# Ryan-Faulkner/Simultaneous-Diffusion-for-Pointclouds

Hardware: AMD Instinct MI355X
Metric: Langevin denoising steps/sec on 64×1024 range images, 1/2/4/8 MI355X (higher is better)
Workload: dtype fp32x3; 1 GPU; Line.yml simultaneous sampling step (score-net fwd + Langevin update + consistency merge), 64x1024x2 range images; views_per_gpu=4, megabatch_views=4, mode=viewsplit, conv_arithmetic=fp32x3, parallelism=views1

## Files before the change

simultaneous-diffusion-for-pointclouds_amd/csrc/conv_kernel.h:

```cpp
#pragma once
#include <type_traits>

#include "common.h"

namespace sdp {

#ifndef SDP_KO
#define SDP_KO 0
#endif

#ifndef SDP_DMA_AUX
#define SDP_DMA_AUX 0
#endif
#ifndef SDP_STORE_AUX
#define SDP_STORE_AUX 0
#endif
#ifndef SDP_STORE_AUX16
#define SDP_STORE_AUX16 SDP_STORE_AUX
#endif

#ifndef SDP_S2_RING
#define SDP_S2_RING 4
#endif

#ifndef SDP_ROWS
#define SDP_ROWS 1
#endif

#ifdef SDP_TIMING
#define SDP_T(i) do { if (tid == 0) tclk[i] = __builtin_amdgcn_s_memtime(); } while (0)
#else
#define SDP_T(i) do { } while (0)
#endif

constexpr int PSTRIDE = 144;

template <int WM, int TC, int KS, int NW = 4, int NJ = 4, bool IO16 = false>
struct ConvTile {
  static constexpr int NTH = 64 * NW;
  static constexpr int WN = NW / WM;
  static constexpr int RW = 128 / TC;
  static constexpr int TR = WM * RW;
  static constexpr int NTILE = WN * 16 * NJ;
  static constexpr int WPC = 4 * (NJ == 2 ? 2 : 1) / NW;
  static constexpr int HALO = KS == 3 ? 1 : 0;
  static constexpr int PC = TC + 2 * HALO;
  static constexpr int PR = TR + 2 * HALO;
  static constexpr int NPIX = PR * PC;
  static constexpr int UPP = IO16 ? 4 : 8;
  static constexpr int NU = (NPIX * UPP + NTH - 1) / NTH;
  static constexpr int PATCH_BYTES = NU * (NTH / UPP) * PSTRIDE;
  static constexpr int RAW_BYTES = NU * NTH * 16;
  static constexpr int PIPE_BYTES = 2 * PATCH_BYTES + RAW_BYTES;
  static constexpr int EPI_BYTES = WM * 64 * (NTILE + 8) * 4;
  static constexpr int LDS_BYTES = PIPE_BYTES > EPI_BYTES ? PIPE_BYTES : EPI_BYTES;
  static_assert(LDS_BYTES * WPC <= 160 * 1024, "LDS budget (WPC workgroups per CU)");
};

SDP_DEV float4 ld4(const float* p) { return *reinterpret_cast<const float4*>(p); }

template <int NU, int NT, int NSTG_ = 5>
struct XformPlan {
  static constexpr int tap_of(int k) { return k * NT / NU; }
  static constexpr int first(int tap) {
    int k = 0;
    while (k < NU && tap_of(k) < tap) ++k;
    return k;
  }
  static constexpr int count(int tap) {
    int n = 0;
    for (int k = 0; k < NU; ++k) n += tap_of(k) == tap ? 1 : 0;
    return n;
  }
  static constexpr int max_count() {
    int m = 0;
    for (int t = 0; t < NT; ++t) m = count(t) > m ? count(t) : m;
    return m;
  }
  static constexpr int NSTG = NSTG_;
// ... 18 lines not shown
    if (kw < 2 && (blk == 8 || blk == 10)) return 4 * 0 + 2 * (blk == 10 ? 1 : 0) + 1;
  } else {
    if (kw < 2 && blk >= 4) return 4 * (1 + (blk - 4) / 2) + 2 * lo + 1;
  }
  return -1;
}
constexpr bool rows_plan_ok() {
  for (int kw = 0; kw < 3; ++kw)
    for (int row = 0; row < 10; ++row)
      for (int lo = 0; lo < 2; ++lo) {
        int n = (kw == 0 && row < 4) ? 1 : 0, at = -1;
        for (int o = 0; o < 9; ++o)
          for (int blk = 0; blk < 16; ++blk) {
            const int c = rows_read(o, blk);
            if (c >= 0 && o / 3 + (c & 1) == kw && c / 4 == row && ((c >> 1) & 1) == lo) {
              ++n;
              at = 16 * o + blk;
            }
          }
        if (n != 1) return false;
        const int kh0 = row > 7 ? row - 7 : 0, mb0 = row - kh0;
        if (at >= 16 * (3 * kw + kh0) + (mb0 < 4 ? mb0 : 4 + mb0)) return false;
        const int pkw = row == 9 ? kw : kw - 1, prow = row == 9 ? 0 : row + 1;
        if (pkw < 0) continue;
        if (rows_slot(pkw, prow) != rows_slot(kw, row)) return false;
        const int kh1 = prow < 2 ? prow : 2, mb1 = prow - kh1;
        if (at < 16 * (3 * pkw + kh1) + (mb1 < 4 ? 4 + mb1 : 8 + mb1)) return false;
      }
  return true;
}
static_assert(rows_plan_ok(), "A-fragment ring: a row is read once, between its slot's last use and its own first");

template <int MODE, int WM, int TC, int KS, bool POOL, bool ZP, bool PELU, int SH = 32, int NW = 4, bool TRN = false,
          int NJ = 4, bool IO16 = false, bool S2 = false>
__global__ __launch_bounds__(64 * NW, NJ == 2 ? 2 : 1) void conv_mfma_kernel(ConvArgs a) {
#if defined(__HIP_DEVICE_COMPILE__)
  static_assert(!IO16 || MODE == MODE_BF16, "the bf16 tape runs in bf16 mode");
  constexpr int ES = IO16 ? 2 : 4;
  constexpr int CPU = IO16 ? 8 : 4;
  constexpr int USH = IO16 ? 2 : 3;
  constexpr int PPU = CPU / 2;
  constexpr bool COPY = IO16 && !PELU;
  static_assert((SH == 32) == (MODE == MODE_F32), "bf16 modes: 16x16 shape; exact fp32: 32x32");
  static_assert(NW == 4 || (SH == 16 && !POOL), "2-wave workgroups: the 16x16 non-pooled forward only");
  static_assert(NJ == 4 || (SH == 16 && !POOL && KS == 3 && WM == 1), "32-Cout waves: the 16x16 3x3 tiles only");
  static_assert(!S2 || (NJ == 2 && NW == 4 && TC == 16 && ZP && !TRN && !IO16), "4x4 stride-2: zero-padded 32-Cout-wave tiles");
  using T = ConvTile<WM, TC, KS, NW, NJ, IO16>;
  constexpr int NTH = T::NTH;
  constexpr int NT = S2 ? 4 : KS * KS;
  constexpr bool TRANS = TRN && SH == 16 && !POOL;
  constexpr int NU = T::NU;
  constexpr int XT = NT >= 4 ? 4 : NT;
  constexpr bool ROWS = SDP_ROWS && SH == 16 && !S2 && NT == 9 && TC == 16 && NJ == 2 && !TRANS;
  __shared__ __attribute__((aligned(16))) char lds[T::LDS_BYTES];
  char* const raw = lds + 2 * T::PATCH_BYTES;

  const int tid = threadIdx.x, lane = tid & 63, wave = tid >> 6;
#ifdef SDP_TIMING
  unsigned long long tclk[8] = {0, 0, 0, 0, 0, 0, 0, 0};
  unsigned long long tbar = 0;
  const unsigned long long rt0 = __builtin_amdgcn_s_memrealtime();
#endif
  SDP_T(0);
  const int wm = WM == 1 ? 0 : (wave & 1), wn = WM == 1 ? wave : (wave >> 1);
  const int d = S2 ? 2 : a.dil, Hs = a.H / d, Ws = a.W / d;
  const int tiles_c = Ws / TC, tiles_rc = (Hs / T::TR) * tiles_c;
  const int nwg = gridDim.x;
  int t = (nwg & 7) ? (int)blockIdx.x : ((int)blockIdx.x & 7) * (nwg >> 3) + ((int)blockIdx.x >> 3);
  const int cblk = a.cpair ? (t & 1) : (int)blockIdx.y;
  if (a.cpair) t >>= 1;
  const int b = t / a.tiles_per_img;
  const int tile = t - b * a.tiles_per_img;
  t = tile;
  const int ph = t / tiles_rc;
  t -= ph * tiles_rc;
  const int ph_r = ph / d, ph_c = ph - (ph / d) * d;
  int trow, tcol;
  if (a.strip_w) {
    const int R = Hs / T::TR, sw = a.strip_w;
    const int strip = t / (R * sw), w_ = t - strip * (R * sw);
    trow = w_ / sw;
    tcol = strip * sw + (w_ - trow * sw);
  } else {
    trow = t / tiles_c;
    tcol = t % tiles_c;
  }
  const int sr0 = trow * T::TR, sc0 = tcol * TC;
  const int n0 = cblk * T::NTILE;
  const int wrow0 = wm * T::RW;

  const int Cin = a.Cin, Cout = a.Cout;
  const int nck = Cin / 32;
  const int nchunks = S2 ? 4 * nck : nck;
  const int NB = Cout / 32;
  const int f0 = n0 / 16 + wn * NJ;
  const int nbg0 = f0 / 2;

  f32x16 acc[4][2];
  f32x4 acc4[8][NJ];
  if constexpr (SH == 32) {
    static_for<0, 4>([&](auto i) {
      static_for<0, 2>([&](auto j) {
#pragma unroll
        for (int r = 0; r < 16; ++r) acc[i][j][r] = 0.f;
      });
    });
// ... 53 lines not shown
    if constexpr (S2) return (c >= 2 * nck ? c - 2 * nck : c) >> 1;
    else return c;
  };
  auto chunk_soff = [&](int c) __attribute__((always_inline)) {
    if constexpr (S2) {
      c = min(c, nchunks - 1);
      const int rho = c >= 2 * nck ? 1 : 0, r = c - rho * 2 * nck;
      return ((rho * a.W + (r & 1)) * Cin + (r >> 1) * 32) * ES;
    } else {
      return c * 32 * ES;
    }
  };
  const int my_cv = tid & (T::UPP - 1);
  float4 ssv[2][PPU];
  auto load_ss = [&](auto buf, int chunk) __attribute__((always_inline)) {
    constexpr int SB = decltype(buf)::value;
    if constexpr (!PELU) return;
    static_for<0, PPU>([&](auto kc) { ssv[SB][kc] = ld4(ssb + (chunk * 32 + my_cv * CPU) * 2 + 4 * decltype(kc)::value); });
  };

  const __amdgpu_buffer_rsrc_t irs =
      __builtin_amdgcn_make_buffer_rsrc((void*)inb, 0, a.H * a.W * Cin * ES, 0x00020000);
  int uoff[NU];
  unsigned uvalid = 0;
  static_for<0, NU>([&](auto kc) {
    constexpr int k = decltype(kc)::value;
    int u = tid + k * NTH;
    bool valid = u < T::NPIX * T::UPP;
    u = valid ? u : 0;
    const int pix = u >> USH, cv = u & (T::UPP - 1);
    const int pr = pix / T::PC, pc = pix - pr * T::PC;
    int sr = sr0 - T::HALO + pr, sc = sc0 - T::HALO + pc;
    if (a.circular) {
      sr = sr < 0 ? sr + Hs : (sr >= Hs ? sr - Hs : sr);
      sc = sc < 0 ? sc + Ws : (sc >= Ws ? sc - Ws : sc);
    } else {
      valid = valid && sr >= 0 && sr < Hs && sc >= 0 && sc < Ws;
      sr = min(max(sr, 0), Hs - 1);
      sc = min(max(sc, 0), Ws - 1);
    }
    const int y = sr * d + ph_r, x = sc * d + ph_c;
    uoff[k] = ((y * a.W + x) * Cin + cv * CPU) * ES;
    uvalid |= (valid ? 1u : 0u) << k;
  });
  auto load_unit = [&](auto kc, int chunk) __attribute__((always_inline)) {
    constexpr int k = decltype(kc)::value;
    if constexpr (SDP_KO & 1) return;
    const int base = __builtin_amdgcn_readfirstlane(((tid & ~63) + k * NTH) * 16);
    __builtin_amdgcn_raw_ptr_buffer_load_lds(
        irs, reinterpret_cast<__attribute__((address_space(3))) void*>(reinterpret_cast<uintptr_t>(raw + base)), 16,
        uoff[k], chunk_soff(chunk), 0, SDP_DMA_AUX);
  };
  const i32x4 irs_o = buffer_desc(inb, (uint32_t)(a.H * a.W * Cin * ES));
  auto load_unit_o = [&](auto kc, int chunk) __attribute__((always_inline)) {
    constexpr int k = decltype(kc)::value;
    if constexpr (SDP_KO & 1) return;
    const uint32_t base = (uint32_t)(uintptr_t)(raw + ((tid & ~63) + k * NTH) * 16);
    dma16_lds_opaque(irs_o, base, uoff[k], chunk_soff(chunk));
  };
  auto xform_load = [&](auto kc) __attribute__((always_inline)) {
    constexpr int k = decltype(kc)::value;
    return *reinterpret_cast<const float4*>(raw + (tid + k * NTH) * 16);
  };
  auto xform_store = [&](auto kc, auto pb, float4 v) __attribute__((always_inline)) {
    constexpr int k = decltype(kc)::value;
    constexpr int PB = decltype(pb)::value;
    const int pix = (tid + k * NTH) >> USH;
    if constexpr (COPY) {
      uint4 u = __builtin_bit_cast(uint4, v);
      if constexpr (ZP) {
        if (!((uvalid >> k) & 1u)) u = make_uint4(0u, 0u, 0u, 0u);
      }
      *reinterpret_cast<uint4*>(lds + PB * T::PATCH_BYTES + pix * PSTRIDE + my_cv * 16) = u;
      return;
    }
    if constexpr (IO16) {
      const uint4 u = __builtin_bit_cast(uint4, v);
      const float4 lo = bf4_to_f4(make_uint2(u.x, u.y)), hi = bf4_to_f4(make_uint2(u.z, u.w));
      float x8[8] = {lo.x, lo.y, lo.z, lo.w, hi.x, hi.y, hi.z, hi.w};
#pragma unroll
      for (int e = 0; e < 8; ++e) {
        if constexpr (PELU) {
          const float4 sv = ssv[PB][e >> 1];
          x8[e] = elu_max(fmaf(x8[e], (e & 1) ? sv.z : sv.x, (e & 1) ? sv.w : sv.y));
        }
        if constexpr (ZP) {
          if (!((uvalid >> k) & 1u)) x8[e] = 0.f;
        }
      }
      *reinterpret_cast<uint4*>(lds + PB * T::PATCH_BYTES + pix * PSTRIDE + my_cv * 16) =
          make_uint4(pack_bf2(x8[0], x8[1]), pack_bf2(x8[2], x8[3]), pack_bf2(x8[4], x8[5]), pack_bf2(x8[6], x8[7]));
      return;
    }
    if constexpr (PELU) {
      const float4 ssv0 = ssv[PB][0], ssv1 = ssv[PB][1];
      v.x = fmaf(v.x, ssv0.x, ssv0.y);
      v.y = fmaf(v.y, ssv0.z, ssv0.w);
      v.z = fmaf(v.z, ssv1.x, ssv1.y);
      v.w = fmaf(v.w, ssv1.z, ssv1.w);
      v.x = elu_max(v.x); v.y = elu_max(v.y); v.z = elu_max(v.z); v.w = elu_max(v.w);
    }
    if constexpr (ZP) {
      if (!((uvalid >> k) & 1u)) v = make_float4(0.f, 0.f, 0.f, 0.f);
    }
    char* dst = lds + PB * T::PATCH_BYTES + pix * PSTRIDE;
    if constexpr (MODE == MODE_F32) {
      *reinterpret_cast<float4*>(dst + my_cv * 16) = v;
    } else {
      bf16x4 hi;
      hi[0] = (__bf16)v.x; hi[1] = (__bf16)v.y; hi[2] = (__bf16)v.z; hi[3] = (__bf16)v.w;
      *reinterpret_cast<bf16x4*>(dst + my_cv * 8) = hi;
// ... 151 lines not shown
        constexpr int NBLK = 8 * NJ;
        static_for<0, NBLK>([&](auto blk_c) {
          constexpr int blk = decltype(blk_c)::value;
          {
            constexpr int s = blk / (4 * NJ), nj = (blk / 4) % NJ, i = blk & 3, mb = 4 * s + i;
            const uint4 h4 = bq[CUR][nj >> 1][2 * (nj & 1)], l4 = bq[CUR][nj >> 1][2 * (nj & 1) + 1];
            const bf16x8 bhi = *reinterpret_cast<const bf16x8*>(&h4);
            const bf16x8 blo = *reinterpret_cast<const bf16x8*>(&l4);
            const bf16x8 ahi = s == 0 ? c0_hi[i] : c1_hi[i];
            if constexpr (TRANS) {
              if constexpr (MODE == MODE_F32X3) {
                const bf16x8 alo = s == 0 ? c0_lo[i] : c1_lo[i];
                acc4[mb][nj] = __builtin_amdgcn_mfma_f32_16x16x32_bf16(bhi, alo, acc4[mb][nj], 0, 0, 0);
                acc4[mb][nj] = __builtin_amdgcn_mfma_f32_16x16x32_bf16(blo, ahi, acc4[mb][nj], 0, 0, 0);
              }
              acc4[mb][nj] = __builtin_amdgcn_mfma_f32_16x16x32_bf16(bhi, ahi, acc4[mb][nj], 0, 0, 0);
            } else {
              if constexpr (MODE == MODE_F32X3) {
                const bf16x8 alo = s == 0 ? c0_lo[i] : c1_lo[i];
                acc4[mb][nj] = __builtin_amdgcn_mfma_f32_16x16x32_bf16(alo, bhi, acc4[mb][nj], 0, 0, 0);
                acc4[mb][nj] = __builtin_amdgcn_mfma_f32_16x16x32_bf16(ahi, blo, acc4[mb][nj], 0, 0, 0);
              }
              acc4[mb][nj] = __builtin_amdgcn_mfma_f32_16x16x32_bf16(ahi, bhi, acc4[mb][nj], 0, 0, 0);
            }
          }
          if constexpr (COPY) {
            if constexpr (blk < NX) xform_store(std::integral_constant<int, tap + XT * blk>{}, std::integral_constant<int, 1 - P>{},
                                                xv[blk]);
          } else if constexpr (blk < PPU * NX) {
            xform_piece(std::integral_constant<int, tap + XT * (blk / PPU)>{}, std::integral_constant<int, blk % PPU>{},
                        std::integral_constant<int, 1 - P>{}, xv[blk / PPU]);
          }
          __builtin_amdgcn_sched_barrier(0);
        });
        if constexpr (NT == 1) dmas();
      }
    });
#ifdef SDP_TIMING
    const unsigned long long tb0 = __builtin_amdgcn_s_memtime();
#endif
    __builtin_amdgcn_s_waitcnt(0xc07f);
    if constexpr (!(SDP_KO & 8)) __builtin_amdgcn_s_barrier();
#ifdef SDP_TIMING
    tbar += __builtin_amdgcn_s_memtime() - tb0;
#endif
  };
  using XP = XformPlan<NU, NT, (MODE == MODE_BF16 && !IO16 && !S2) ? 8 : 5>;
  constexpr int NQ = MODE == MODE_F32X3 ? 8 : 4;
  constexpr int NWL = NJ * (MODE == MODE_F32X3 ? 2 : 1);
  constexpr int NBLK = 8 * NJ;
  static_assert(NQ <= NBLK / 2 && 2 * NWL <= NBLK, "the tap's fillers fit its blocks");
  using I0 = std::integral_constant<int, 0>;
  using I1 = std::integral_constant<int, 1>;
  auto read_a1 = [&](const char* pat, auto pos_c, auto s_c, auto i_c, auto lo_c) __attribute__((always_inline)) {
    constexpr int pos = decltype(pos_c)::value, s = decltype(s_c)::value, i = decltype(i_c)::value;
    constexpr int kh = pos / 3, kw = pos % 3, mb = 4 * s + i;
    constexpr int mr = mb / (TC / 16), mc = (mb % (TC / 16)) * 16;
    return *reinterpret_cast<const bf16x8*>(pat + ((wrow0 + mr + kh) * T::PC + mc + kw) * PSTRIDE + a_lane_off16 +
                                            (decltype(lo_c)::value ? 64 : 0));
  };
  auto load_b1 = [&](auto buf, auto q_c, int chunk, int tap) __attribute__((always_inline)) {
    constexpr int J = decltype(buf)::value, q = decltype(q_c)::value;
    constexpr int nj = MODE == MODE_F32X3 ? (q >> 1) : q, part = MODE == MODE_F32X3 ? (q & 1) : 0;
    if constexpr (SDP_KO & 4) return;
    const int so = __builtin_amdgcn_readfirstlane(((chunk * NT + tap) * NB) * 4096 + (part ? wlo16 : 0));
    const u32x4 v = __builtin_amdgcn_raw_buffer_load_b128(wrs, wq16[nj], so, 0);
    bq[J][nj >> 1][2 * (nj & 1) + part] = make_uint4(v.x, v.y, v.z, v.w);
  };
  auto do_chunk9 = [&](auto parity, auto phase_c, int chunk) __attribute__((always_inline)) {
    constexpr int P = decltype(parity)::value, PHS = decltype(phase_c)::value;
    const char* pat = lds + P * T::PATCH_BYTES;
    bf16x8 ca[2][4], cb[2][4];
    bf16x8 ar[2][ROWS ? ROWS_SLOTS : 1];
    auto read_row = [&](auto kw_c, auto row_c, auto lo_c) __attribute__((always_inline)) {
      return *reinterpret_cast<const bf16x8*>(pat + ((wrow0 + decltype(row_c)::value) * T::PC + decltype(kw_c)::value) * PSTRIDE +
                                              a_lane_off16 + (decltype(lo_c)::value ? 64 : 0));
    };
    static_for<0, 4>([&](auto i) {
      if constexpr (ROWS) {
        ar[0][rows_slot(0, i)] = read_row(I0{}, i, I0{});
        if constexpr (MODE == MODE_F32X3) ar[1][rows_slot(0, i)] = read_row(I0{}, i, I1{});
      } else {
        using POS0 = std::integral_constant<int, S2 ? s2_pos(PHS, 0) : 0>;
        ca[0][i] = read_a1(pat, POS0{}, I0{}, i, I0{});
        if constexpr (MODE == MODE_F32X3) ca[1][i] = read_a1(pat, POS0{}, I0{}, i, I1{});
      }
    });
    load_ss(std::integral_constant<int, P>{}, chunk_cc(min(chunk + 2, nchunks - 1)));
    static_for<0, NT>([&](auto tap_c) {
      constexpr int tap = decltype(tap_c)::value;
      constexpr int DIST = NBUF - 1;
      constexpr int CUR = tap % NBUF, NXT = (tap + DIST) % NBUF;
      using POS = std::integral_constant<int, S2 ? s2_pos(PHS, tap) : tap>;
      using POSN = std::integral_constant<int, S2 ? s2_pos(PHS, tap + 1 < NT ? tap + 1 : 0) : tap + 1>;
      constexpr int U0 = XP::first(tap), UN = XP::count(tap), Q = COPY ? UN : UN * PPU * XP::NSTG;
      constexpr int UNA = UN > 0 ? UN : 1;
      const int wchunk = tap + DIST < NT ? chunk : min(chunk + 1, nchunks - 1);
      constexpr int wnext = tap + DIST < NT ? tap + DIST : tap + DIST - NT;
      constexpr int wtap = ROWS ? rows_pos(wnext) : wnext;
      float4 xr[UNA];
      float py0[PPU * UNA], py1[PPU * UNA], pe0[PPU * UNA], pe1[PPU * UNA];
      uint32_t phi[PPU * UNA], plo[PPU * UNA];
      auto stage = [&](auto pc_c, auto st_c) __attribute__((always_inline)) {
        constexpr int pc = decltype(pc_c)::value, st = decltype(st_c)::value;
        constexpr int j = pc / PPU, h = pc % PPU, k = U0 + j, PB = 1 - P;
        if constexpr (SDP_KO & 2) return;
        if constexpr (COPY) {
          xform_store(std::integral_constant<int, U0 + decltype(pc_c)::value>{}, std::integral_constant<int, PB>{},
                      xr[decltype(pc_c)::value]);
          return;
        }
        auto raw2 = [&](float& r0, float& r1) __attribute__((always_inline)) {
          const float4 v = xr[j];
          if constexpr (IO16) {
            const uint32_t w = __float_as_uint(h == 0 ? v.x : h == 1 ? v.y : h == 2 ? v.z : v.w);
            r0 = __uint_as_float(w << 16);
            r1 = __uint_as_float(w & 0xffff0000u);
          } else {
            r0 = h ? v.z : v.x;
            r1 = h ? v.w : v.y;
          }
        };
        if constexpr (XP::NSTG == 8) {
          const float4 v = xr[j];
          if constexpr (st == 0) {
            py0[pc] = h ? v.z : v.x;
            if constexpr (PELU) {
              py0[pc] = fmaf(py0[pc], ssv[PB][h].x, ssv[PB][h].y);
              pe0[pc] = fminf(py0[pc], 0.f);
            }
          } else if constexpr (st == 1) {
            py1[pc] = h ? v.w : v.y;
            if constexpr (PELU) {
              py1[pc] = fmaf(py1[pc], ssv[PB][h].z, ssv[PB][h].w);
              pe1[pc] = fminf(py1[pc], 0.f);
            }
          } else if constexpr (st == 2) {
            if constexpr (PELU) pe0[pc] = __expf(pe0[pc]);
          } else if constexpr (st == 3) {
            if constexpr (PELU) pe1[pc] = __expf(pe1[pc]);
          } else if constexpr (st == 4) {
// ... 13 lines not shown
            *reinterpret_cast<uint32_t*>(lds + PB * T::PATCH_BYTES + pix * PSTRIDE + my_cv * 8 + h * 4) = phi[pc];
          }
          return;
        }
        if constexpr (st == 0) {
          float r0, r1;
          raw2(r0, r1);
          py0[pc] = r0;
          py1[pc] = r1;
          if constexpr (PELU) {
            const float4 sv = ssv[PB][h];
            py0[pc] = fmaf(r0, sv.x, sv.y);
            py1[pc] = fmaf(r1, sv.z, sv.w);
            pe0[pc] = fminf(py0[pc], 0.f);
            pe1[pc] = fminf(py1[pc], 0.f);
          }
        } else if constexpr (st == 1) {
          if constexpr (PELU) {
            pe0[pc] = __expf(pe0[pc]);
            pe1[pc] = __expf(pe1[pc]);
          }
        } else if constexpr (st == 2) {
          if constexpr (PELU) {
            py0[pc] = fmaxf(py0[pc], pe0[pc] - 1.0f);
            py1[pc] = fmaxf(py1[pc], pe1[pc] - 1.0f);
          }
          if constexpr (ZP) {
            const bool ok = (uvalid >> k) & 1u;
            py0[pc] = ok ? py0[pc] : 0.f;
            py1[pc] = ok ? py1[pc] : 0.f;
          }
        } else if constexpr (st == 3) {
          typedef __attribute__((ext_vector_type(2))) __bf16 bf16x2;
          bf16x2 hi;
          hi[0] = (__bf16)py0[pc];
          hi[1] = (__bf16)py1[pc];
          phi[pc] = *reinterpret_cast<const uint32_t*>(&hi);
          if constexpr (MODE == MODE_F32X3) {
            bf16x2 lo;
            lo[0] = (__bf16)(py0[pc] - (float)hi[0]);
            lo[1] = (__bf16)(py1[pc] - (float)hi[1]);
            plo[pc] = *reinterpret_cast<const uint32_t*>(&lo);
          }
        } else {
          const int pix = (tid + k * NTH) >> USH;
          char* dst = lds + PB * T::PATCH_BYTES + pix * PSTRIDE + my_cv * (2 * CPU) + h * 4;
          *reinterpret_cast<uint32_t*>(dst) = phi[pc];
          if constexpr (MODE == MODE_F32X3) *reinterpret_cast<uint32_t*>(dst + 64) = plo[pc];
        }
      };
      static_for<0, NBLK>([&](auto blk_c) {
        constexpr int blk = decltype(blk_c)::value;
        constexpr int s = blk / (4 * NJ), nj = (blk / 4) % NJ, i = blk & 3, mb = 4 * s + i;
        if constexpr (blk < UN) xr[blk] = xform_load(std::integral_constant<int, U0 + blk>{});
        {
          const uint4 h4 = bq[CUR][nj >> 1][2 * (nj & 1)], l4 = bq[CUR][nj >> 1][2 * (nj & 1) + 1];
          const bf16x8 bhi = *reinterpret_cast<const bf16x8*>(&h4);
          const bf16x8 blo = *reinterpret_cast<const bf16x8*>(&l4);
          auto afrag = [&](auto lo_c) __attribute__((always_inline)) {
            constexpr int lo = decltype(lo_c)::value;
            if constexpr (ROWS) return ar[lo][rows_slot(tap / 3, mb + tap % 3)];
            else return s == 0 ? ca[lo][i] : cb[lo][i];
          };
          const bf16x8 ahi = afrag(I0{});
          if constexpr (TRANS) {
            if constexpr (MODE == MODE_F32X3) {
              const bf16x8 alo = afrag(I1{});
              acc4[mb][nj] = __builtin_amdgcn_mfma_f32_16x16x32_bf16(bhi, alo, acc4[mb][nj], 0, 0, 0);
              acc4[mb][nj] = __builtin_amdgcn_mfma_f32_16x16x32_bf16(blo, ahi, acc4[mb][nj], 0, 0, 0);
            }
            acc4[mb][nj] = __builtin_amdgcn_mfma_f32_16x16x32_bf16(bhi, ahi, acc4[mb][nj], 0, 0, 0);
          } else {
            if constexpr (MODE == MODE_F32X3) {
              const bf16x8 alo = afrag(I1{});
              acc4[mb][nj] = __builtin_amdgcn_mfma_f32_16x16x32_bf16(alo, bhi, acc4[mb][nj], 0, 0, 0);
              acc4[mb][nj] = __builtin_amdgcn_mfma_f32_16x16x32_bf16(ahi, blo, acc4[mb][nj], 0, 0, 0);
            }
            acc4[mb][nj] = __builtin_amdgcn_mfma_f32_16x16x32_bf16(ahi, bhi, acc4[mb][nj], 0, 0, 0);
          }
        }
        if constexpr (ROWS) {
          constexpr int c = rows_read(tap, blk);
          if constexpr (c >= 0 && (MODE == MODE_F32X3 || !(c & 2)))
            ar[(c >> 1) & 1][rows_slot(tap / 3 + (c & 1), c / 4)] = read_row(std::integral_constant<int, tap / 3 + (c & 1)>{}, std::integral_constant<int, c / 4>{},
                                               std::integral_constant<int, (c >> 1) & 1>{});
        } else if constexpr (blk < NQ) {
          constexpr int q = blk, ii = MODE == MODE_F32X3 ? (q >> 1) : q, lo = MODE == MODE_F32X3 ? (q & 1) : 0;
          cb[lo][ii] = read_a1(pat, POS{}, I1{}, std::integral_constant<int, ii>{}, std::integral_constant<int, lo>{});
        }
        if constexpr ((blk & 1) && (blk >> 1) < NWL)
          load_b1(std::integral_constant<int, NXT>{}, std::integral_constant<int, (blk >> 1)>{}, wchunk, wtap);
        if constexpr (!ROWS && tap + 1 < NT && blk >= NBLK / 2 && blk < NBLK / 2 + NQ) {
          constexpr int q = blk - NBLK / 2, ii = MODE == MODE_F32X3 ? (q >> 1) : q, lo = MODE == MODE_F32X3 ? (q & 1) : 0;
          ca[lo][ii] = read_a1(pat, POSN{}, I0{}, std::integral_constant<int, ii>{},
                               std::integral_constant<int, lo>{});
        }
        static_for<0, Q>([&](auto q_c) {
          constexpr int q = decltype(q_c)::value;
          if constexpr (XP::stage_blk(q, Q, NBLK) == blk) {
            if constexpr (COPY) stage(std::integral_constant<int, q>{}, std::integral_constant<int, 0>{});
            else stage(std::integral_constant<int, q / XP::NSTG>{}, std::integral_constant<int, q % XP::NSTG>{});
          }
        });
        if constexpr (UN > 0 && blk >= NBLK - UN)
          load_unit_o(std::integral_constant<int, U0 + blk - (NBLK - UN)>{}, chunk + 2);
        __builtin_amdgcn_sched_barrier(0);
      });
    });
    __builtin_amdgcn_s_waitcnt(0xc07f);
    if constexpr (!(SDP_KO & 8)) __builtin_amdgcn_s_barrier();
  };
  static_assert(NT % 2 == 1 || (S2 && NT % NBUF == 0), "weight-ring slots repeat from chunk to chunk");
#ifndef SDP_DGRAD16_TAPS
#define SDP_DGRAD16_TAPS 0
#endif
  if constexpr (S2) {
    static_assert(MODE != MODE_F32 && NT % NBUF == 0, "4x4 stride-2: the tap schedule of the bf16 modes");
    static_assert(XP::max_count() * PPU * XP::NSTG <= 2 * (NBLK - 2), "at most two transform stages per block");
    for (int chunk = 0; chunk < 2 * nck; chunk += 2) {
      do_chunk9(I0{}, I0{}, chunk);
      do_chunk9(I1{}, I1{}, chunk + 1);
    }
    for (int chunk = 2 * nck; chunk < nchunks; chunk += 2) {
      do_chunk9(I0{}, std::integral_constant<int, 2>{}, chunk);
      do_chunk9(I1{}, std::integral_constant<int, 3>{}, chunk + 1);
    }
  } else if constexpr (MODE != MODE_F32 && NT == 9 && (!TRANS || (IO16 && SDP_DGRAD16_TAPS))) {
    static_assert(XP::max_count() * PPU * XP::NSTG <= 2 * (NBLK - 2), "at most two transform stages per block");
    for (int chunk = 0; chunk < nchunks; chunk += 2) {
      do_chunk9(I0{}, I0{}, chunk);
      do_chunk9(I1{}, I0{}, chunk + 1);
    }
  } else {
    for (int chunk = 0; chunk < nchunks; chunk += 2) {
      do_chunk(std::integral_constant<int, 0>{}, chunk);
      do_chunk(std::integral_constant<int, 1>{}, chunk + 1);
    }
  }

  SDP_T(3);
  if (TRANS && (!a.dact || TC < 32 || NW != 4)) {
    if constexpr (TRANS) {
    __builtin_amdgcn_s_waitcnt(0);
    const int Ho = a.H, Wo = a.W;
    const size_t bo = (size_t)b * Ho * Wo * Cout;
    const int img_bytes = Ho * Wo * Cout * ES;
    auto rs = [&](const float* p) {
      return __builtin_amdgcn_make_buffer_rsrc((void*)(reinterpret_cast<const char*>(p) + bo * ES), 0, img_bytes, 0x00020000);
    };
    const int lq = lane >> 4, lcol = lane & 15;
    constexpr int CB = TC / 16;
    const int voff = (lcol * d * Cout + 4 * lq) * ES;
    auto soff = [&](int mb, int nj) {
      const int mr = mb / CB, mc = (mb % CB) * 16;
      const int y = (sr0 + wrow0 + mr) * d + ph_r, x = (sc0 + mc) * d + ph_c;
      return __builtin_amdgcn_readfirstlane(((y * Wo + x) * Cout + n0 + wn * 16 * NJ + nj * 16) * ES);
    };
    auto ld = [&](__amdgpu_buffer_rsrc_t r, int so) {
      if constexpr (IO16) {
        typedef __attribute__((ext_vector_type(2))) unsigned u32x2;
        const u32x2 q = __builtin_amdgcn_raw_buffer_load_b64(r, voff, so, 0);
        return bf4_to_f4(make_uint2(q.x, q.y));
      } else {
        const u32x4 q = __builtin_amdgcn_raw_buffer_load_b128(r, voff, so, 0);
        return make_float4(__uint_as_float(q.x), __uint_as_float(q.y), __uint_as_float(q.z), __uint_as_float(q.w));
      }
    };
    auto st = [&](float4 v, __amdgpu_buffer_rsrc_t r, int so, auto aux_c) {
      constexpr int AUX = decltype(aux_c)::value;
      if constexpr (IO16) {
        typedef __attribute__((ext_vector_type(2))) unsigned u32x2;
        const uint2 w = f4_to_bf4(v);
        __builtin_amdgcn_raw_buffer_store_b64(u32x2{w.x, w.y}, r, voff, so, AUX);
      } else {
        const u32x4 q = {__float_as_uint(v.x), __float_as_uint(v.y), __float_as_uint(v.z), __float_as_uint(v.w)};
        __builtin_amdgcn_raw_buffer_store_b128(q, r, voff, so, AUX);
      }
    };
    auto rs_or_out = [&](const float* p) { return rs(p ? p : a.out); };
    const __amdgpu_buffer_rsrc_t ors = rs(a.out), xrs = rs_or_out(a.aux), rrs = rs_or_out(a.res), o2rs = rs_or_out(a.out2),
                                 r2rs = rs_or_out(a.res2);
    static_for<0, NJ>([&](auto njc) {
      constexpr int nj = decltype(njc)::value;
      __builtin_amdgcn_sched_barrier(0);
      const int co0 = n0 + wn * 16 * NJ + nj * 16 + 4 * lq;
      float4 hq[8], rq[8], s0 = make_float4(1.f, 0.f, 1.f, 0.f), s1 = s0;
      if (a.dact) static_for<0, 8>([&](auto mb) { hq[mb] = ld(xrs, soff(mb, nj)); });
      if (a.dact == 3) {
        s0 = ld4(a.epi_ss + ((size_t)b * Cout + co0) * 2);
        s1 = ld4(a.epi_ss + ((size_t)b * Cout + co0) * 2 + 4);
      }
      if (a.res) static_for<0, 8>([&](auto mb) { rq[mb] = ld(rrs, soff(mb, nj)); });
      const float4 bias4 = a.bias ? ld4(a.bias + co0) : make_float4(0.f, 0.f, 0.f, 0.f);
      const float4 esc = make_float4(s0.x, s0.z, s1.x, s1.z), esh = make_float4(s0.y, s0.w, s1.y, s1.w);
      float4 v[8];
      static_for<0, 8>([&](auto mbc) {
// ... 54 lines not shown
      if (a.epi_elu) {
#pragma unroll
        for (int mb = 0; mb < 8; ++mb) v[mb] = make_float4(elu(v[mb].x), elu(v[mb].y), elu(v[mb].z), elu(v[mb].w));
      }
      if constexpr (!(SDP_KO & 16)) {
        static_for<0, 8>([&](auto mbc) {
          constexpr int mb = decltype(mbc)::value;
          st(v[mb], ors, soff(mb, nj), std::integral_constant<int, IO16 ? SDP_STORE_AUX16 : SDP_STORE_AUX>{});
        });
      }
      if (a.stats) {
        float mean[4], m2[4];
        static_for<0, 4>([&](auto rc) {
          constexpr int r = decltype(rc)::value;
          auto comp = [&](const float4& q) { return r == 0 ? q.x : r == 1 ? q.y : r == 2 ? q.z : q.w; };
          float s = 0.f;
#pragma unroll
          for (int mb = 0; mb < 8; ++mb) s += comp(v[mb]);
          mean[r] = s * 0.125f;
          float q2 = 0.f;
#pragma unroll
          for (int mb = 0; mb < 8; ++mb) {
            const float dv = comp(v[mb]) - mean[r];
            q2 = fmaf(dv, dv, q2);
          }
          m2[r] = q2;
        });
        auto merge = [&](auto ctl_c, float n) {
          constexpr int CTL = decltype(ctl_c)::value;
#pragma unroll
          for (int r = 0; r < 4; ++r) {
            const float mp = __int_as_float(__builtin_amdgcn_mov_dpp(__float_as_int(mean[r]), CTL, 0xf, 0xf, false));
            const float qp = __int_as_float(__builtin_amdgcn_mov_dpp(__float_as_int(m2[r]), CTL, 0xf, 0xf, false));
            const float dm = mean[r] - mp;
            m2[r] = m2[r] + qp + dm * dm * (0.5f * n);
            mean[r] = 0.5f * (mean[r] + mp);
          }
        };
        merge(std::integral_constant<int, 0xB1>{}, 8.f);
        merge(std::integral_constant<int, 0x4E>{}, 16.f);
        merge(std::integral_constant<int, 0x141>{}, 32.f);
        merge(std::integral_constant<int, 0x140>{}, 64.f);
        if (lcol == 0) {
          float4* sp = reinterpret_cast<float4*>(reinterpret_cast<float2*>(a.stats) +
                                                 ((size_t)b * a.groups_per_img + tile * WM + wm) * Cout + co0);
          sp[0] = make_float4(mean[0], m2[0], mean[1], m2[1]);
          sp[1] = make_float4(mean[2], m2[2], mean[3], m2[3]);
        }
      }
    });
    }
  } else if (SH == 16 && !TRANS && (!a.dact || TC < 32 || NW != 4)) {
    if constexpr (SH == 16 && !TRANS) {
    __builtin_amdgcn_s_waitcnt(0);
    const int Ho = (POOL || S2) ? a.H / 2 : a.H, Wo = (POOL || S2) ? a.W / 2 : a.W;
    const int de = S2 ? 1 : d;
    const size_t bo = (size_t)b * Ho * Wo * Cout;
    const int img_bytes = Ho * Wo * Cout * ES;
    auto rs = [&](const float* p) {
      return __builtin_amdgcn_make_buffer_rsrc((void*)(reinterpret_cast<const char*>(p ? p : a.out) + bo * ES), 0, img_bytes,
                                               0x00020000);
    };
    const __amdgpu_buffer_rsrc_t ors = rs(a.out), rrs = rs(a.res), o2rs = rs(a.out2), r2rs = rs(a.res2), xrs = rs(a.aux);
    const int lq = lane >> 4, lcol = lane & 15;
    constexpr int CB = TC / 16;
    constexpr int NF = POOL ? CB : 8;
    constexpr int PER = POOL ? 2 : 4;
    constexpr int NV = NF * PER;
    const int xs = (POOL ? 1 : de) * Cout * ES;
    int vbase[NF];
    static_for<0, NF>([&](auto fc) {
      constexpr int f = decltype(fc)::value;
      const int co = n0 + wn * 16 * NJ + lcol;
      if constexpr (POOL) {
        vbase[f] = (((sr0 >> 1) * Wo + ((sc0 + f * 16) >> 1) + 2 * lq) * Cout + co) * ES;
      } else {
        constexpr int mr = f / CB, mc = (f % CB) * 16;
        const int y = (sr0 + wrow0 + mr) * de + ph_r, x = (sc0 + mc + 4 * lq) * de + ph_c;
        vbase[f] = ((y * Wo + x) * Cout + co) * ES;
      }
    });
#define SDP_EPI16_OFF(i, nj) vbase[(i) / PER], __builtin_amdgcn_readfirstlane(((i) % PER) * xs + (nj) * 16 * ES)
    auto ld1 = [&](__amdgpu_buffer_rsrc_t r, int vo, int so) __attribute__((always_inline)) {
      if constexpr (IO16) return __uint_as_float((uint32_t)__builtin_amdgcn_raw_buffer_load_b16(r, vo, so, 0) << 16);
      else return __uint_as_float(__builtin_amdgcn_raw_buffer_load_b32(r, vo, so, 0));
    };
    auto store_vals = [&](const float (&w)[NV], __amdgpu_buffer_rsrc_t r, auto nj_c, auto aux_c) __attribute__((always_inline)) {
      constexpr int NJC = decltype(nj_c)::value, AUX = decltype(aux_c)::value;
      if constexpr (IO16) {
        constexpr int HP = PER / 2;
        const bool odd = lane & 1;
#pragma unroll
        for (int f = 0; f < NF; ++f) {
          const int vb = vbase[f] + (odd ? HP * xs - 2 : 0);
#pragma unroll
          for (int k = 0; k < HP; ++k) {
            const float mine = odd ? w[f * PER + HP + k] : w[f * PER + k];
            const float send = odd ? w[f * PER + k] : w[f * PER + HP + k];
            const float got = __int_as_float(__builtin_amdgcn_mov_dpp(__float_as_int(send), 0xB1, 0xf, 0xf, false));
            const uint32_t pk = odd ? pack_bf2(got, mine) : pack_bf2(mine, got);
            __builtin_amdgcn_raw_buffer_store_b32(pk, r, vb, __builtin_amdgcn_readfirstlane(k * xs + NJC * 16 * ES), AUX);
          }
        }
      } else {
#pragma unroll
        for (int i = 0; i < NV; ++i) __builtin_amdgcn_raw_buffer_store_b32(__float_as_uint(w[i]), r, SDP_EPI16_OFF(i, NJC), AUX);
      }
// ... 60 lines not shown
          float h = ld1(xrs, SDP_EPI16_OFF(i, nj));
          if (a.dact == 3) h = fmaf(h, esc, esh);
          v[i] = v[i] * elu_grad(h, a.dact);
        }
      }
      if (a.res) {
#pragma unroll
        for (int i = 0; i < NV; ++i) v[i] = pre[nj][i] + v[i];
      }
      if (a.out2) {
        float r2[NV];
#pragma unroll
        for (int i = 0; i < NV; ++i)
          r2[i] = a.res ? ld1(r2rs, SDP_EPI16_OFF(i, nj)) : pre[nj][i];
#pragma unroll
        for (int i = 0; i < NV; ++i) r2[i] = v[i] + r2[i];
        store_vals(r2, o2rs, njc, std::integral_constant<int, 0>{});
      }
      if (a.epi_elu) {
#pragma unroll
        for (int i = 0; i < NV; ++i) v[i] = elu(v[i]);
      }
      if constexpr (!(SDP_KO & 16))
        store_vals(v, ors, njc, std::integral_constant<int, IO16 ? SDP_STORE_AUX16 : SDP_STORE_AUX>{});
      if (a.stats) {
        float sum = 0.f;
#pragma unroll
        for (int i = 0; i < NV; ++i) sum += v[i];
        float mean = sum * (1.0f / NV);
        float m2 = 0.f;
#pragma unroll
        for (int i = 0; i < NV; ++i) {
          const float dv = v[i] - mean;
          m2 = fmaf(dv, dv, m2);
        }
        float mp = __shfl_xor(mean, 16), qp = __shfl_xor(m2, 16), dm = mean - mp;
        m2 = m2 + qp + dm * dm * (0.5f * NV);
        mean = 0.5f * (mean + mp);
        mp = __shfl_xor(mean, 32);
        qp = __shfl_xor(m2, 32);
        dm = mean - mp;
        m2 = m2 + qp + dm * dm * (float)NV;
        mean = 0.5f * (mean + mp);
        if (lq == 0) {
          float2* st = reinterpret_cast<float2*>(a.stats) + ((size_t)b * a.groups_per_img + tile * WM + wm) * Cout + co;
          *st = make_float2(mean, m2);
        }
      }
    });
#undef SDP_EPI16_OFF
    }
  } else if (a.dact) {
    if constexpr (TC >= 32 && NW == 4 && SH == 16) {
    __builtin_amdgcn_s_waitcnt(0);
    __syncthreads();
    constexpr int SROW = T::NTILE + 8;
    constexpr int SP = WM * 64;
    constexpr int CG = T::NTILE / 4;
    constexpr int PL = 256 / CG;
    constexpr int NPO = POOL ? SP / 4 : SP;
    static_assert(SP * SROW * 4 <= T::LDS_BYTES, "epilogue staging fits the LDS");
    float* stage = reinterpret_cast<float*>(lds);
    const int cg = tid % CG, pl = tid / CG;
    const int co0 = n0 + cg * 4;
    const float4 bias4 = a.bias ? ld4(a.bias + co0) : make_float4(0.f, 0.f, 0.f, 0.f);
    float4 es0 = make_float4(1.f, 0.f, 1.f, 0.f), es1 = es0;
    if (a.dact == 3) {
      es0 = ld4(a.epi_ss + ((size_t)b * Cout + co0) * 2);
      es1 = ld4(a.epi_ss + ((size_t)b * Cout + co0) * 2 + 4);
    }
    const int Ho = POOL ? a.H / 2 : a.H, Wo = POOL ? a.W / 2 : a.W;
    using TA = std::conditional_t<IO16, __bf16, float>;
    auto tp = [](const float* p) { return reinterpret_cast<const TA*>(p); };
    TA* const outb = reinterpret_cast<TA*>(a.out) + (size_t)b * Ho * Wo * Cout;
    float4 sK[WM], s1[WM], s2[WM];
    int sn[WM];
    static_for<0, WM>([&](auto g) {
      sK[g] = make_float4(0.f, 0.f, 0.f, 0.f); s1[g] = sK[g]; s2[g] = sK[g]; sn[g] = 0;
    });
    static_for<0, 2>([&](auto hc) {
      constexpr int h = decltype(hc)::value;
      {
        if constexpr (!POOL && TRANS) {
          static_for<0, 4>([&](auto ic) {
            constexpr int i = decltype(ic)::value;
            static_for<0, 4>([&](auto njc) {
              constexpr int nj = decltype(njc)::value;
              float* dst = stage + (wm * 64 + 16 * i + (lane & 15)) * SROW + wn * 64 + nj * 16 + 4 * (lane >> 4);
              const f32x4 q = acc4[4 * h + i][nj];
              *reinterpret_cast<float4*>(dst) = make_float4(q[0], q[1], q[2], q[3]);
            });
          });
        } else if constexpr (!POOL) {
          static_for<0, 4>([&](auto ic) {
            constexpr int i = decltype(ic)::value;
            static_for<0, 4>([&](auto njc) {
              constexpr int nj = decltype(njc)::value;
              float* dst = stage + (wm * 64 + 16 * i + 4 * (lane >> 4)) * SROW + wn * 64 + nj * 16 + (lane & 15);
  #pragma unroll
              for (int r = 0; r < 4; ++r) dst[r * SROW] = acc4[4 * h + i][nj][r];
            });
          });
        }
      }
      __syncthreads();
      auto pix = [&](int j, int& y, int& x, int& g) __attribute__((always_inline)) {
        if constexpr (POOL) {
// ... 278 lines not shown
```

Before: 395.7 image-steps/s.

## Peel the last two conv chunks to drop redundant prefetches and waits

Adds a tail mode to the 9-tap and stride-2 conv main loops. The last two chunks are peeled into specialised instances that skip the input DMA, scale/shift, transform-stage and out-of-range weight prefetches that would fetch clamped, already-loaded data. The final chunk also skips its barrier and the epilogue's full waitcnt when the staged epilogue does not need it. The wave-uniform LDS base for the opaque DMA is hoisted out of the per-unit lambda. This cuts wasted memory traffic and synchronisation in the pipeline drain, but it risks correctness if any outstanding load is still needed by the epilogue.

```diff
diff --git a/simultaneous-diffusion-for-pointclouds_amd/csrc/conv_kernel.h b/simultaneous-diffusion-for-pointclouds_amd/csrc/conv_kernel.h
--- a/simultaneous-diffusion-for-pointclouds_amd/csrc/conv_kernel.h
+++ b/simultaneous-diffusion-for-pointclouds_amd/csrc/conv_kernel.h
@@ -25,6 +25,14 @@
 
 #ifndef SDP_ROWS
 #define SDP_ROWS 1
+#endif
+
+#ifndef SDP_TAIL
+#define SDP_TAIL 1
+#endif
+
+#ifndef SDP_DGRAD16_TAPS
+#define SDP_DGRAD16_TAPS 0
 #endif
 
 #ifdef SDP_TIMING
@@ -149,6 +157,9 @@
   constexpr int NU = T::NU;
   constexpr int XT = NT >= 4 ? 4 : NT;
   constexpr bool ROWS = SDP_ROWS && SH == 16 && !S2 && NT == 9 && TC == 16 && NJ == 2 && !TRANS;
+  constexpr bool TAPS9 = S2 || (MODE != MODE_F32 && NT == 9 && (!TRANS || (IO16 && SDP_DGRAD16_TAPS)));
+  constexpr bool TAILED = SDP_TAIL && TAPS9;
+  constexpr bool STAGED_EPI = TC >= 32 && NW == 4 && SH == 16;
   __shared__ __attribute__((aligned(16))) char lds[T::LDS_BYTES];
   char* const raw = lds + 2 * T::PATCH_BYTES;
 
@@ -308,11 +319,11 @@
         uoff[k], chunk_soff(chunk), 0, SDP_DMA_AUX);
   };
   const i32x4 irs_o = buffer_desc(inb, (uint32_t)(a.H * a.W * Cin * ES));
+  const uint32_t raw_wave = (uint32_t)__builtin_amdgcn_readfirstlane((int)(uint32_t)(uintptr_t)(raw + (tid & ~63) * 16));
   auto load_unit_o = [&](auto kc, int chunk) __attribute__((always_inline)) {
     constexpr int k = decltype(kc)::value;
     if constexpr (SDP_KO & 1) return;
-    const uint32_t base = (uint32_t)(uintptr_t)(raw + ((tid & ~63) + k * NTH) * 16);
-    dma16_lds_opaque(irs_o, base, uoff[k], chunk_soff(chunk));
+    dma16_lds_opaque(irs_o, raw_wave + k * NTH * 16, uoff[k], chunk_soff(chunk));
   };
   auto xform_load = [&](auto kc) __attribute__((always_inline)) {
     constexpr int k = decltype(kc)::value;
@@ -570,6 +581,8 @@
   static_assert(NQ <= NBLK / 2 && 2 * NWL <= NBLK, "the tap's fillers fit its blocks");
   using I0 = std::integral_constant<int, 0>;
   using I1 = std::integral_constant<int, 1>;
+  using I2 = std::integral_constant<int, 2>;
+  using I3 = std::integral_constant<int, 3>;
   auto read_a1 = [&](const char* pat, auto pos_c, auto s_c, auto i_c, auto lo_c) __attribute__((always_inline)) {
     constexpr int pos = decltype(pos_c)::value, s = decltype(s_c)::value, i = decltype(i_c)::value;
     constexpr int kh = pos / 3, kw = pos % 3, mb = 4 * s + i;
@@ -585,8 +598,8 @@
     const u32x4 v = __builtin_amdgcn_raw_buffer_load_b128(wrs, wq16[nj], so, 0);
     bq[J][nj >> 1][2 * (nj & 1) + part] = make_uint4(v.x, v.y, v.z, v.w);
   };
-  auto do_chunk9 = [&](auto parity, auto phase_c, int chunk) __attribute__((always_inline)) {
-    constexpr int P = decltype(parity)::value, PHS = decltype(phase_c)::value;
+  auto do_chunk9 = [&](auto parity, auto phase_c, int chunk, auto tail_c) __attribute__((always_inline)) {
+    constexpr int P = decltype(parity)::value, PHS = decltype(phase_c)::value, TAIL = decltype(tail_c)::value;
     const char* pat = lds + P * T::PATCH_BYTES;
     bf16x8 ca[2][4], cb[2][4];
     bf16x8 ar[2][ROWS ? ROWS_SLOTS : 1];
@@ -604,7 +617,8 @@
         if constexpr (MODE == MODE_F32X3) ca[1][i] = read_a1(pat, POS0{}, I0{}, i, I1{});
       }
     });
-    load_ss(std::integral_constant<int, P>{}, chunk_cc(min(chunk + 2, nchunks - 1)));
+    if constexpr (TAIL == 0)
+      load_ss(std::integral_constant<int, P>{}, chunk_cc(min(chunk + 2, nchunks - 1)));
     static_for<0, NT>([&](auto tap_c) {
       constexpr int tap = decltype(tap_c)::value;
       constexpr int DIST = NBUF - 1;
@@ -724,7 +738,7 @@
       static_for<0, NBLK>([&](auto blk_c) {
         constexpr int blk = decltype(blk_c)::value;
         constexpr int s = blk / (4 * NJ), nj = (blk / 4) % NJ, i = blk & 3, mb = 4 * s + i;
-        if constexpr (blk < UN) xr[blk] = xform_load(std::integral_constant<int, U0 + blk>{});
+        if constexpr (TAIL < 2 && blk < UN) xr[blk] = xform_load(std::integral_constant<int, U0 + blk>{});
         {
           const uint4 h4 = bq[CUR][nj >> 1][2 * (nj & 1)], l4 = bq[CUR][nj >> 1][2 * (nj & 1) + 1];
           const bf16x8 bhi = *reinterpret_cast<const bf16x8*>(&h4);
@@ -760,48 +774,55 @@
           constexpr int q = blk, ii = MODE == MODE_F32X3 ? (q >> 1) : q, lo = MODE == MODE_F32X3 ? (q & 1) : 0;
           cb[lo][ii] = read_a1(pat, POS{}, I1{}, std::integral_constant<int, ii>{}, std::integral_constant<int, lo>{});
         }
-        if constexpr ((blk & 1) && (blk >> 1) < NWL)
+        if constexpr ((blk & 1) && (blk >> 1) < NWL && (TAIL < 2 || tap + DIST < NT))
           load_b1(std::integral_constant<int, NXT>{}, std::integral_constant<int, (blk >> 1)>{}, wchunk, wtap);
         if constexpr (!ROWS && tap + 1 < NT && blk >= NBLK / 2 && blk < NBLK / 2 + NQ) {
           constexpr int q = blk - NBLK / 2, ii = MODE == MODE_F32X3 ? (q >> 1) : q, lo = MODE == MODE_F32X3 ? (q & 1) : 0;
           ca[lo][ii] = read_a1(pat, POSN{}, I0{}, std::integral_constant<int, ii>{},
                                std::integral_constant<int, lo>{});
         }
-        static_for<0, Q>([&](auto q_c) {
+        static_for<0, (TAIL < 2 ? Q : 0)>([&](auto q_c) {
           constexpr int q = decltype(q_c)::value;
           if constexpr (XP::stage_blk(q, Q, NBLK) == blk) {
             if constexpr (COPY) stage(std::integral_constant<int, q>{}, std::integral_constant<int, 0>{});
             else stage(std::integral_constant<int, q / XP::NSTG>{}, std::integral_constant<int, q % XP::NSTG>{});
           }
         });
-        if constexpr (UN > 0 && blk >= NBLK - UN)
+        if constexpr (TAIL == 0 && UN > 0 && blk >= NBLK - UN)
           load_unit_o(std::integral_constant<int, U0 + blk - (NBLK - UN)>{}, chunk + 2);
         __builtin_amdgcn_sched_barrier(0);
       });
     });
-    __builtin_amdgcn_s_waitcnt(0xc07f);
-    if constexpr (!(SDP_KO & 8)) __builtin_amdgcn_s_barrier();
+    if constexpr (TAIL < 2 || STAGED_EPI) {
+      __builtin_amdgcn_s_waitcnt(0xc07f);
+      if constexpr (!(SDP_KO & 8)) __builtin_amdgcn_s_barrier();
+    }
   };
   static_assert(NT % 2 == 1 || (S2 && NT % NBUF == 0), "weight-ring slots repeat from chunk to chunk");
-#ifndef SDP_DGRAD16_TAPS
-#define SDP_DGRAD16_TAPS 0
-#endif
   if constexpr (S2) {
     static_assert(MODE != MODE_F32 && NT % NBUF == 0, "4x4 stride-2: the tap schedule of the bf16 modes");
     static_assert(XP::max_count() * PPU * XP::NSTG <= 2 * (NBLK - 2), "at most two transform stages per block");
     for (int chunk = 0; chunk < 2 * nck; chunk += 2) {
-      do_chunk9(I0{}, I0{}, chunk);
-      do_chunk9(I1{}, I1{}, chunk + 1);
-    }
-    for (int chunk = 2 * nck; chunk < nchunks; chunk += 2) {
-      do_chunk9(I0{}, std::integral_constant<int, 2>{}, chunk);
-      do_chunk9(I1{}, std::integral_constant<int, 3>{}, chunk + 1);
-    }
-  } else if constexpr (MODE != MODE_F32 && NT == 9 && (!TRANS || (IO16 && SDP_DGRAD16_TAPS))) {
+      do_chunk9(I0{}, I0{}, chunk, I0{});
+      do_chunk9(I1{}, I1{}, chunk + 1, I0{});
+    }
+    for (int chunk = 2 * nck; chunk < nchunks - (TAILED ? 2 : 0); chunk += 2) {
+      do_chunk9(I0{}, I2{}, chunk, I0{});
+      do_chunk9(I1{}, I3{}, chunk + 1, I0{});
+    }
+    if constexpr (TAILED) {
+      do_chunk9(I0{}, I2{}, nchunks - 2, I1{});
+      do_chunk9(I1{}, I3{}, nchunks - 1, I2{});
+    }
+  } else if constexpr (TAPS9) {
     static_assert(XP::max_count() * PPU * XP::NSTG <= 2 * (NBLK - 2), "at most two transform stages per block");
-    for (int chunk = 0; chunk < nchunks; chunk += 2) {
-      do_chunk9(I0{}, I0{}, chunk);
-      do_chunk9(I1{}, I0{}, chunk + 1);
+    for (int chunk = 0; chunk < nchunks - (TAILED ? 2 : 0); chunk += 2) {
+      do_chunk9(I0{}, I0{}, chunk, I0{});
+      do_chunk9(I1{}, I0{}, chunk + 1, I0{});
+    }
+    if constexpr (TAILED) {
+      do_chunk9(I0{}, I0{}, nchunks - 2, I1{});
+      do_chunk9(I1{}, I0{}, nchunks - 1, I2{});
     }
   } else {
     for (int chunk = 0; chunk < nchunks; chunk += 2) {
@@ -813,7 +834,7 @@
   SDP_T(3);
   if (TRANS && (!a.dact || TC < 32 || NW != 4)) {
     if constexpr (TRANS) {
-    __builtin_amdgcn_s_waitcnt(0);
+    if constexpr (!TAILED) __builtin_amdgcn_s_waitcnt(0);
     const int Ho = a.H, Wo = a.W;
     const size_t bo = (size_t)b * Ho * Wo * Cout;
     const int img_bytes = Ho * Wo * Cout * ES;
@@ -974,7 +995,7 @@
     }
   } else if (SH == 16 && !TRANS && (!a.dact || TC < 32 || NW != 4)) {
     if constexpr (SH == 16 && !TRANS) {
-    __builtin_amdgcn_s_waitcnt(0);
+    if constexpr (!TAILED) __builtin_amdgcn_s_waitcnt(0);
     const int Ho = (POOL || S2) ? a.H / 2 : a.H, Wo = (POOL || S2) ? a.W / 2 : a.W;
     const int de = S2 ? 1 : d;
     const size_t bo = (size_t)b * Ho * Wo * Cout;
@@ -1141,7 +1162,7 @@
     }
   } else if (a.dact) {
     if constexpr (TC >= 32 && NW == 4 && SH == 16) {
-    __builtin_amdgcn_s_waitcnt(0);
+    if constexpr (!TAILED) __builtin_amdgcn_s_waitcnt(0);
     __syncthreads();
     constexpr int SROW = T::NTILE + 8;
     constexpr int SP = WM * 64;
```

Measured after the change: 402.4 image-steps/s, median of 6. +1.7%, better.
